# orjfickel/Small-Project-UV-Robot-Ray-Tracer

Hardware: AMD Instinct MI355X
Metric: Mray/s (extend+shade) on C046_1.glb 1920x1080x8-bounce (higher is better)
Workload: dtype f32; 1 GPU; testroomopt.glb (stand-in for the absent rooms/C046_1.glb), 2073600 photons/launch x 8 waves, lamp 0 of lange_route.xml, SEED_0=0; step = reset + generate + extend of all waves (batched), accumulate + shade replayed per wave + sync; triangles=44866, mode=batched, launch_pipelining=True, flavour=0, seed_mode=0, wide_bvh=False, parallelism=1 GPU, self_comm=False, high_priority_stream=False, full=False

## Files before the change

include/uvrt.h:

```cpp
#ifndef UVRT_H
#define UVRT_H

#include <stdint.h>

#ifdef __cplusplus
extern "C" {
#endif

typedef struct uvrt_ctx uvrt_ctx;

enum {
    UVRT_OK = 0,
    UVRT_ERR_INVALID = -1,
    UVRT_ERR_HIP = -2,
    UVRT_ERR_NO_DEVICE = -3,
    UVRT_ERR_BVH = -4,
    UVRT_ERR_STACK = -5
};

enum { UVRT_MAP_SUM = 0, UVRT_MAP_MAX = 1 };

const char* uvrt_last_error(void);
const char* uvrt_version(void);

// ... 96 lines not shown
int32_t uvrt_dedupe_classes_default(void);
int uvrt_batch_deposits(uvrt_ctx* ctx, int64_t* out);
int uvrt_batch_residue(uvrt_ctx* ctx, int64_t* nonzero);
int uvrt_dedupe_classes(const float lamp[3], int32_t count, const uint32_t* seed_prev, const uint32_t* seed_next,
                        int32_t seed_mode, int64_t first_gid, int64_t n, int32_t max_classes, uint32_t* class_masks,
                        int32_t* class_count, int64_t* deposits);
int uvrt_set_helper_priority(uvrt_ctx* ctx, int32_t prio);
int uvrt_get_helper_priority(uvrt_ctx* ctx, int32_t* prio);
int uvrt_batch_traced_rays(uvrt_ctx* ctx, int64_t* out);
uint32_t uvrt_seed_input(int64_t gid, const float lamp[3], uint32_t seed_prev, uint32_t seed_next, int32_t seed_mode);
int uvrt_dedupe_plan(const float lamp[3], int32_t count, const uint32_t* seed_prev, const uint32_t* seed_next,
                     int32_t seed_mode, int64_t first_gid, int64_t n, uint32_t* masks);
int uvrt_dedupe_plan_tiled(const float lamp[3], int32_t count, const uint32_t* seed_prev, const uint32_t* seed_next,
                           int32_t seed_mode, int64_t first_gid, int64_t n, int32_t tile_keys, int64_t chunk_first,
                           int64_t chunk_n, uint32_t* masks);
int uvrt_dedupe_mark_device(uvrt_ctx* ctx, const float lamp[3], int32_t count, const uint32_t* seed_prev,
                            const uint32_t* seed_next, int32_t seed_mode, int64_t first_gid, int64_t n, int64_t chunk_first,
                            int64_t chunk_n, uint32_t* masks, uint32_t* block_owner_counts);

int uvrt_comm_available(void);
int uvrt_comm_unique_id(void* id128);
int uvrt_comm_init_rank(uvrt_ctx* ctx, const void* id128, int32_t rank, int32_t world);
int uvrt_comm_init_all(uvrt_ctx** ctxs, int32_t n);
int uvrt_comm_destroy(uvrt_ctx* ctx);
int uvrt_comm_info(uvrt_ctx* ctx, int32_t out4[4]);
int uvrt_reduce_batch(uvrt_ctx* ctx);
int uvrt_reduce_batch_group(uvrt_ctx** ctxs, int32_t n);

enum { UVRT_PLAN_CONVERGED = 0, UVRT_PLAN_ITERATION_CAP = 1 };
typedef struct {
// ... 84 lines not shown
```

small-project-uv-robot-ray-tracer_amd/capi.py:

```python
from __future__ import annotations

import ctypes as C
import os

import numpy as np

_HERE = os.path.dirname(os.path.abspath(__file__))
LIB_PATH = os.path.join(_HERE, "libuvrt_hip.so")
LIB_DEV_PATH = os.path.join(_HERE, "libuvrt_hip_dev.so")

RAY_DT = np.dtype([("dirx", "<f4"), ("diry", "<f4"), ("dirz", "<f4"),
                   ("origx", "<f4"), ("origy", "<f4"), ("origz", "<f4"),
                   ("dist", "<f4"), ("triID", "<u4")])

MAP_SUM, MAP_MAX = 0, 1

_vp, _i32, _i64, _f32, _u32 = C.c_void_p, C.c_int32, C.c_int64, C.c_float, C.c_uint32
_fp = C.POINTER(C.c_float)
SYMBOLS = [
    ("uvrt_last_error", C.c_char_p, []),
    ("uvrt_version", C.c_char_p, []),
    ("uvrt_create", C.c_int, [C.c_int, C.POINTER(_vp)]),
    ("uvrt_destroy", None, [_vp]),
    ("uvrt_set_stream", C.c_int, [_vp, _vp]),
# ... 18 lines not shown
    ("uvrt_fold_batch", C.c_int, [_vp]),
    ("uvrt_read_batch_counts", C.c_int, [_vp, _i32, _vp, _i32, _i32]),
    ("uvrt_set_dedupe", C.c_int, [_vp, _i32]),
    ("uvrt_set_helper_priority", C.c_int, [_vp, _i32]),
    ("uvrt_get_helper_priority", C.c_int, [_vp, C.POINTER(_i32)]),
    ("uvrt_batch_traced_rays", C.c_int, [_vp, C.POINTER(_i64)]),
    ("uvrt_set_dedupe_classes", C.c_int, [_vp, _i32]),
    ("uvrt_get_dedupe_classes", C.c_int, [_vp, C.POINTER(_i32)]),
    ("uvrt_dedupe_classes_default", _i32, []),
    ("uvrt_batch_deposits", C.c_int, [_vp, C.POINTER(_i64)]),
    ("uvrt_batch_residue", C.c_int, [_vp, C.POINTER(_i64)]),
    ("uvrt_dedupe_classes", C.c_int, [_fp, _i32, _vp, _vp, _i32, _i64, _i64, _i32, _vp, C.POINTER(_i32), C.POINTER(_i64)]),
    ("uvrt_seed_input", _u32, [_i64, _fp, _u32, _u32, _i32]),
    ("uvrt_dedupe_plan", C.c_int, [_fp, _i32, _vp, _vp, _i32, _i64, _i64, _vp]),
    ("uvrt_dedupe_plan_tiled", C.c_int, [_fp, _i32, _vp, _vp, _i32, _i64, _i64, _i32, _i64, _i64, _vp]),
    ("uvrt_dedupe_mark_device", C.c_int, [_vp, _fp, _i32, _vp, _vp, _i32, _i64, _i64, _i64, _i64, _vp, _vp]),
    ("uvrt_comm_available", C.c_int, []),
    ("uvrt_comm_info", C.c_int, [_vp, C.POINTER(_i32)]),
    ("uvrt_comm_unique_id", C.c_int, [_vp]),
    ("uvrt_comm_init_rank", C.c_int, [_vp, _vp, _i32, _i32]),
    ("uvrt_comm_init_all", C.c_int, [C.POINTER(_vp), _i32]),
    ("uvrt_comm_destroy", C.c_int, [_vp]),
    ("uvrt_reduce_batch", C.c_int, [_vp]),
    ("uvrt_reduce_batch_group", C.c_int, [C.POINTER(_vp), _i32]),
    ("uvrt_advance_seed", C.c_int, [_vp, _fp, _f32]),
    ("uvrt_set_seed_mode", C.c_int, [_vp, _i32]),
    ("uvrt_seed_next_mode", _u32, [_fp, _f32, _u32, _i32]),
    ("uvrt_set_sort_bits", C.c_int, [_vp, _i32]),
    ("uvrt_set_record_hits", C.c_int, [_vp, _i32]),
    ("uvrt_set_flavour", C.c_int, [_vp, _i32]),
# ... 172 lines not shown
    sn = np.ascontiguousarray(seed_next_, dtype=np.uint32)
    assert sp.size == sn.size
    max_classes = dedupe_classes_default() if max_classes is None else max_classes
    out = np.zeros(DEDUPE_CLASS_MAX, dtype=np.uint32)
    nc, dep = _i32(), _i64()
    rc = lib().uvrt_dedupe_classes(_f3(lamp), int(sp.size), _ptr(sp), _ptr(sn), int(seed_mode), int(first_gid), int(n),
                                   int(max_classes), _ptr(out), C.byref(nc), C.byref(dep))
    if rc != 0:
        raise UvrtError("uvrt error %d: %s" % (rc, lib().uvrt_last_error().decode()))
    return out[:int(nc.value)].copy(), int(dep.value)


DEDUPE_CLASS_MAX = 32
DEDUPE_CLASS_LAUNCHES = 30
DEDUPE_TILE_KEYS = 3840
DEDUPE_BLOCK_GIDS = 2048


def dedupe_plan_tiled(lamp, seed_prev, seed_next_, seed_mode, first_gid, n, tile_keys=DEDUPE_TILE_KEYS, chunk_first=None,
                      chunk_n=None):
    sp = np.ascontiguousarray(seed_prev, dtype=np.uint32)
    sn = np.ascontiguousarray(seed_next_, dtype=np.uint32)
    assert sp.size == sn.size
    chunk_first = first_gid if chunk_first is None else chunk_first
    chunk_n = n if chunk_n is None else chunk_n
    out = np.empty((sp.size, int(chunk_n)), dtype=np.uint32)
    rc = lib().uvrt_dedupe_plan_tiled(_f3(lamp), int(sp.size), _ptr(sp), _ptr(sn), int(seed_mode), int(first_gid), int(n),
                                      int(tile_keys), int(chunk_first), int(chunk_n), _ptr(out))
    if rc != 0:
        raise UvrtError("uvrt error %d: %s" % (rc, lib().uvrt_last_error().decode()))
    return out


def seed_next_sweep(frm, light_length, seed_prev):
    return int(lib().uvrt_seed_next_sweep(_f3(frm), float(np.float32(light_length)), int(seed_prev)))


def comm_unique_id():
    buf = C.create_string_buffer(128)
    rc = lib().uvrt_comm_unique_id(buf)
    if rc != 0:
        raise UvrtError("uvrt error %d: %s" % (rc, lib().uvrt_last_error().decode()))
    return buf.raw
# ... 463 lines not shown
```

small-project-uv-robot-ray-tracer_amd/csrc/uvrt_capi.hip:

```cpp
#include "uvrt_ctx.h"

using namespace uvrt;
using namespace uvrt_impl;

namespace uvrt_impl {

thread_local std::string g_err;

int fail(int code, const char* fmt, ...)
{
    char buf[512];
    va_list ap;
    va_start(ap, fmt);
    vsnprintf(buf, sizeof buf, fmt, ap);
    va_end(ap);
    g_err = buf;
    return code;
}

}

uvrt_ctx::~uvrt_ctx()
{
    plan_drop(this);
// ... 74 lines not shown
        if (l > 0) HIP_TRY(hipStreamCreateWithFlags(&c->lanes[l].side, hipStreamNonBlocking));
        HIP_TRY(hipEventCreateWithFlags(&c->lanes[l].ev_tail, hipEventDisableTiming));
    }
    HIP_TRY(hipEventCreateWithFlags(&c->ev_fence, hipEventDisableTiming));
    HIP_TRY(hipEventCreateWithFlags(&c->ev_mapfence, hipEventDisableTiming));
    if (const char* e = getenv("UVRT_LANES")) { const int v = atoi(e); if (v >= 1 && v <= uvrt_ctx::MAXL) c->nlanes = v; }
    if (const char* e = getenv("UVRT_PIPELINE")) c->pipeline = atoi(e) != 0;
    if (const char* e = getenv("UVRT_BATCH_CHUNK_MB")) { const long v = atol(e); if (v > 0) c->batch_chunk_bytes = c->dedupe_chunk_bytes = (size_t)v << 20; }
#ifdef UVRT_DEV_VARIANTS
    if (const char* e = getenv("UVRT_PROBE_SKIP_GENERATE")) c->probe_skip_generate = atoi(e);
    if (const char* e = getenv("UVRT_NEARFAR_MINMAX")) c->nearfar_minmax = atoi(e) != 0;
#endif
    if (const char* e = getenv("UVRT_DRAIN_MERGE")) c->drain_merge = atoi(e) != 0;
    if (const char* e = getenv("UVRT_DEDUPE")) c->dedupe = atoi(e) != 0;
    if (const char* e = getenv("UVRT_DEDUPE_CLASSES")) { const int v = atoi(e); if (v >= 0 && v <= DEDUPE_CLASS_MAX) c->dedupe_classes = v; }
    if (const char* e = getenv("UVRT_DEDUPE_CLASS_REPLICAS")) { const int v = atoi(e); if (v >= 1 && v <= 16) c->dedupe_class_replicas = v; }
    if (const char* e = getenv("UVRT_DEDUPE_CLASS_MB")) { const long v = atol(e); if (v > 0 && v <= 4096) c->dedupe_class_bytes = (size_t)v << 20; }
    if (const char* e = getenv("UVRT_HELPER_PRIO")) { const int v = atoi(e); if (v >= 0 && v <= 3) c->helper_prio = v; }
    if (const char* e = getenv("UVRT_BATCH_LANES")) { const int v = atoi(e); if (v >= 1 && v <= uvrt_ctx::MAXL - 1) c->batch_lanes = v; }
    if (const char* e = getenv("UVRT_COMM_RESERVE_CUS")) { const int v = atoi(e); if (v >= 0 && v <= 64 && v % 8 == 0) c->comm_reserve_knob = v; }
    if (const char* e = getenv("UVRT_HOT_SAMPLE")) { const int v = atoi(e); if (v >= 256 && v <= (1 << 20)) c->hot_sample = v; }
    if (const char* e = getenv("UVRT_HOT_DIRECT")) { const int v = atoi(e); if (v >= 0 && v <= 8192) c->hot_direct = v; }
    if (const char* e = getenv("UVRT_HOT_TAIL")) { const int v = atoi(e); if (v >= 0 && v < 64) c->hot_tail = v; }
    if (int rc = c->error_flag.ensure(256, true, c->stream)) return rc;
#ifndef UVRT_TRIP_STATS
    void* dp = nullptr;
    HIP_TRY(hipHostMalloc((void**)&c->host_flag, 64, hipHostMallocMapped | hipHostMallocCoherent));
    HIP_TRY(hipHostGetDevicePointer(&dp, c->host_flag, 0));
    memset(c->host_flag, 0, 64);
    c->host_flag_dev = (uint32_t*)dp;
// ... 624 lines not shown
```

small-project-uv-robot-ray-tracer_amd/csrc/uvrt_capi_batch.hip:

```cpp
#include "uvrt_ctx.h"

using namespace uvrt;
using namespace uvrt_impl;

namespace uvrt_impl {

static int trace_launches(uvrt_ctx* c, const uvrt_launch* launches, float light_length, int32_t count, int64_t first_gid,
                          int64_t n, const char* who)
{
    if (!c || !launches || !c->have_scene) return fail(UVRT_ERR_INVALID, "%s: null argument or no scene", who);
    if (count <= 0 || count > MAX_BATCH) return fail(UVRT_ERR_INVALID, "%s: count must be in [1,%d]", who, MAX_BATCH);
    if (n <= 0 || first_gid < 0 || first_gid + n > (int64_t)INT32_MAX)
        return fail(UVRT_ERR_INVALID, "%s: bad global-id range", who);
    if (c->b_count > 0) return fail(UVRT_ERR_INVALID, "%s: the previous batch has not been replayed (uvrt_replay_batch)", who);
    if (c->record_hits || c->sort_bits != 0)
        return fail(UVRT_ERR_INVALID, "%s: per-ray hit records and ray ordering are per-launch features", who);
    int nsweeps = 0;
    for (int k = 0; k < count; ++k) {
        if (launches[k].kind != UVRT_LAUNCH_STOP && launches[k].kind != UVRT_LAUNCH_SWEEP)
            return fail(UVRT_ERR_INVALID, "%s: launch %d: kind must be UVRT_LAUNCH_STOP or UVRT_LAUNCH_SWEEP", who, k);
        nsweeps += launches[k].kind == UVRT_LAUNCH_SWEEP;
    }
    if (nsweeps > 0 && c->seed_mode != 0)
        return fail(UVRT_ERR_INVALID, "%s: seed mode 1 models the SEED race of generate.cl only; a sweep needs "
// ... 247 lines not shown
            for (int64_t g0 = 0; g0 < n; g0 += pc.chunk_gids) {
                const int64_t gn = std::min(pc.chunk_gids, n - g0);
                const int ph0 = gfirst[g] + pc.k0;
                hipStream_t ls;
                if (int rcl = next_chunk_lane(&ls)) return rcl;
                const size_t at = (size_t)ph0 * (size_t)n_pad + (size_t)pc.kc * (size_t)g0;
                GenDedupeParams dq;
                memset(&dq, 0, sizeof dq);
                dq.g = pc.G;
                dq.rays = S.rays.as<float4>() + at;
                dq.masks = S.masks.as<uint32_t>() + at;
                dq.total = S.dd_counts.as<uint32_t>() + dd_used;
                dq.deposits = S.dd_counts.as<uint32_t>() + dd_chunks + dd_used++;
                dq.cls = pc.cls;
                dq.tmp = cur_lane(c).dd_tmp.as<uint32_t>();
                dq.block_counts = cur_lane(c).dd_blocks.as<uint32_t>();
                dq.g0 = first_gid + g0;
                dq.gn = gn;
                dedupe_tile_range(dq.g, dq.g0, dq.gn, DEDUPE_TILE_KEYS, dq.key_lo, dq.tiles);
                dq.light_length = light_length;
                dq.prio = c->helper_prio;
                launch_generate_dedupe(dq, ls);
                if (int rcl = lane_stream(c, &ls)) return rcl;
                ExtendParams p;
                fill_launch(c, p, gx[g], gz[g]);
                p.rays = dq.rays;
                p.masks = dq.masks;
                p.n_dev = dq.total;
                p.counts = S.planes.as<int32_t>() + (size_t)ph0 * plane_ints;
                p.count_replicas = R;
                p.count_stride = c->T;
                p.n = (int64_t)pc.kc * gn;
                p.plane_stride = (uint32_t)plane_ints;
                p.cls_replicas = pc.cls.count > 0 ? cls_repl : 0;
// ... 201 lines not shown
        return fail(UVRT_ERR_INVALID, "%s: null argument, or count outside [2,%d]", who, DEDUPE_MAX);
    memset(&G, 0, sizeof G);
    G.lx = lamp[0]; G.ly = lamp[1]; G.lz = lamp[2];
    G.seed_mode = seed_mode;
    G.count = count;
    G.first_gid = first_gid; G.n = n;
    for (int j = 0; j < count; ++j) { G.seed_prev[j] = seed_prev[j]; G.seed_next[j] = seed_next[j]; }
    if (!dedupe_group_ok(G)) return fail(UVRT_ERR_INVALID, "%s: these launches cannot form a dedupe group", who);
    return UVRT_OK;
}
static bool chunk_ok(const DedupeGroup& G, int64_t chunk_first, int64_t chunk_n)
{
    return chunk_n > 0 && chunk_first >= G.first_gid && chunk_first + chunk_n <= G.first_gid + G.n;
}

int uvrt_dedupe_plan_tiled(const float lamp[3], int32_t count, const uint32_t* seed_prev, const uint32_t* seed_next,
                           int32_t seed_mode, int64_t first_gid, int64_t n, int32_t tile_keys, int64_t chunk_first,
                           int64_t chunk_n, uint32_t* masks)
{
    DedupeGroup G;
    if (int rc = hook_group(G, "uvrt_dedupe_plan_tiled", lamp, count, seed_prev, seed_next, seed_mode, first_gid, n)) return rc;
    if (!masks || tile_keys <= 0 || !chunk_ok(G, chunk_first, chunk_n))
        return fail(UVRT_ERR_INVALID, "uvrt_dedupe_plan_tiled: null masks, no tile width, or a chunk outside the range");
    std::vector<uint32_t> table((size_t)tile_keys);
    dedupe_plan_tiled(G, tile_keys, chunk_first, chunk_n, table.data(), masks);
    return UVRT_OK;
}

int32_t uvrt_dedupe_classes_default(void) { return DEDUPE_CLASSES_DEFAULT; }

int uvrt_dedupe_classes(const float lamp[3], int32_t count, const uint32_t* seed_prev, const uint32_t* seed_next, int32_t seed_mode,
                        int64_t first_gid, int64_t n, int32_t max_classes, uint32_t* class_masks, int32_t* class_count,
                        int64_t* deposits)
{
    DedupeGroup G;
    if (int rc = hook_group(G, "uvrt_dedupe_classes", lamp, count, seed_prev, seed_next, seed_mode, first_gid, n)) return rc;
    if (!class_masks || !class_count || max_classes < 0 || max_classes > DEDUPE_CLASS_MAX)
        return fail(UVRT_ERR_INVALID, "uvrt_dedupe_classes: null output, or a maximum outside [0,%d]", DEDUPE_CLASS_MAX);
    std::vector<uint32_t> table((size_t)DEDUPE_TILE_KEYS);
    DedupeTally cand[DEDUPE_CLASS_MAX];
    int nc = 0;
// ... 15 lines not shown
{
    if (!c) return fail(UVRT_ERR_INVALID, "uvrt_dedupe_mark_device: null context");
    GenDedupeParams dq;
    memset(&dq, 0, sizeof dq);
    if (int rc = hook_group(dq.g, "uvrt_dedupe_mark_device", lamp, count, seed_prev, seed_next, seed_mode, first_gid, n)) return rc;
    if (!masks || !block_owner_counts || !chunk_ok(dq.g, chunk_first, chunk_n))
        return fail(UVRT_ERR_INVALID, "uvrt_dedupe_mark_device: null output, or a chunk outside the range");
    if (int rc = set_device(c)) return rc;
    if (int rc = join_all(c)) return rc;
    Lane& L = c->lanes[0];
    const size_t nblocks = (size_t)count * (size_t)((chunk_n + DD_SLOTS - 1) / DD_SLOTS);
    HIP_TRY(hipStreamSynchronize(c->stream));
    if (int rc = L.dd_tmp.ensure((size_t)count * (size_t)chunk_n * 4, false, c->stream)) return rc;
    if (int rc = L.dd_blocks.ensure((size_t)count * (size_t)((chunk_n + 255) / 256) * 4, true, c->stream)) return rc;
    dq.tmp = L.dd_tmp.as<uint32_t>();
    dq.block_counts = L.dd_blocks.as<uint32_t>();
    dq.g0 = chunk_first;
    dq.gn = chunk_n;
    dedupe_tile_range(dq.g, dq.g0, dq.gn, DEDUPE_TILE_KEYS, dq.key_lo, dq.tiles);
    dq.prio = c->helper_prio;
    launch_dedupe_mark(dq, c->stream);
    HIP_TRY(hipGetLastError());
    HIP_TRY(hipMemcpyAsync(masks, dq.tmp, (size_t)count * (size_t)chunk_n * 4, hipMemcpyDeviceToHost, c->stream));
    HIP_TRY(hipMemcpyAsync(block_owner_counts, dq.block_counts, nblocks * 4, hipMemcpyDeviceToHost, c->stream));
    HIP_TRY(hipMemsetAsync(dq.block_counts, 0, nblocks * 4, c->stream));
    HIP_TRY(hipStreamSynchronize(c->stream));
    return UVRT_OK;
}

int uvrt_fold_batch(uvrt_ctx* c)
{
    if (!c || c->b_count <= 0) return fail(UVRT_ERR_INVALID, "uvrt_fold_batch: no traced batch");
    if (c->b_is_folded) return UVRT_OK;
    if (int rc = set_device(c)) return rc;
// ... 85 lines not shown
```

small-project-uv-robot-ray-tracer_amd/csrc/uvrt_ctx.h:

```cpp
#pragma once
#include "../../include/uvrt.h"
#include "uvrt_device.h"

#include <cmath>
#include <cstdarg>
#include <cstdio>
#include <cstring>
#include <memory>
#include <string>
#include <vector>

namespace uvrt_impl {

extern thread_local std::string g_err;
int fail(int code, const char* fmt, ...);

#define HIP_TRY(expr)                                                                   \
    do {                                                                                \
        hipError_t e_ = (expr);                                                         \
        if (e_ != hipSuccess)                                                           \
            return ::uvrt_impl::fail(UVRT_ERR_HIP, "%s failed: %s (%s:%d)", #expr,      \
                                     hipGetErrorString(e_), __FILE__, __LINE__);        \
    } while (0)

// ... 115 lines not shown
    uint64_t b_chunks = 0;
    int batch_lanes = 2;
    int32_t b_repl = 16;
    std::vector<DevBuf> b_recs;
    struct RecsKey {
        RecsTag tag; const uint32_t* perm = nullptr; uint64_t gen = 0;
        bool holds(float ox, float oz, const uint32_t* pm, uint64_t g) const { return tag.matches(ox, oz) && perm == pm && gen == g; }
    };
    std::vector<RecsKey> b_recs_key;
    int32_t b_count = 0;
    int64_t b_n = 0, b_npad = 0;
    int32_t b_phys[uvrt::MAX_BATCH] = {};
    int helper_prio = 1;
    bool dedupe = true;
    int64_t b_traced_known = -1;
    int32_t b_traced_chunks = 0;
    int32_t dedupe_classes = uvrt::DEDUPE_CLASSES_DEFAULT;
    int32_t dedupe_class_replicas = 4;
    size_t dedupe_class_bytes = (size_t)96 << 20;
    int32_t b_ncls = 0, b_cls_repl = 1;
    uint64_t b_cls_launches[uvrt::MAX_CLASS_PLANES] = {};
    bool b_is_folded = false;
    void* comm = nullptr;
    int comm_reserve_knob = 8;
    int lanes_masked_cus = 0;
    int comm_rank = 0, comm_world = 1;

    uint32_t seed = 0;
    int32_t seed_mode = 0;

// ... 286 lines not shown
```

small-project-uv-robot-ray-tracer_amd/csrc/uvrt_dedupe.h:

```cpp
#pragma once
#include <stdint.h>

#if defined(__HIPCC__)
#define UVRT_HD __host__ __device__ __forceinline__
#else
#define UVRT_HD inline
#endif

namespace uvrt {

constexpr int DEDUPE_MAX = 31;
constexpr int64_t DEDUPE_GID_END = 126322567;

UVRT_HD float seed_sum_of(int threadID, uint32_t SEED, float lx, float ly, float lz)
{
    float acc = (float)(int)((uint32_t)threadID * 17u + 1u);
    acc = acc + lx * 13.0f;
    acc = acc + ly * 7.0f;
    acc = acc + lz * 11.0f;
    acc = acc + (float)(SEED >> 15);
    return acc;
}
UVRT_HD float seed_sum(int64_t gid, float lx, float ly, float lz, uint32_t seed_prev, uint32_t seed_next, int32_t seed_mode)
{
// ... 10 lines not shown
    float lx, ly, lz;
    int32_t seed_mode;
    int32_t count;
    int64_t first_gid, n;
    uint32_t seed_prev[DEDUPE_MAX], seed_next[DEDUPE_MAX];
    int32_t offset[DEDUPE_MAX];
    int32_t key0[DEDUPE_MAX];
};

UVRT_HD int32_t dedupe_key(const DedupeGroup& G, int j, int64_t gid)
{
    const int32_t s = (int32_t)seed_sum(gid, G.lx, G.ly, G.lz, G.seed_prev[j], G.seed_next[j], G.seed_mode);
    return (G.seed_mode == 1 && s < 0) ? 0 : s;
}

UVRT_HD int32_t dedupe_key1(const DedupeGroup& G, int j, int32_t gid)
{
    const int32_t s = (int32_t)seed_sum_of(gid, G.seed_mode == 1 ? G.seed_prev[j] : G.seed_next[j], G.lx, G.ly, G.lz);
    return (G.seed_mode == 1 && s < 0) ? 0 : s;
}

UVRT_HD int32_t dedupe_find(const DedupeGroup& G, int j, int32_t t, int32_t lo, int32_t last, int32_t& g)
{
    g = g < lo ? lo : (g > last ? last : g);
    int32_t v = dedupe_key1(G, j, g);
    while (v > t && g > lo) v = dedupe_key1(G, j, --g);
    while (v < t && g < last) v = dedupe_key1(G, j, ++g);
    return v;
}
UVRT_HD int32_t dedupe_estimate(const DedupeGroup& G, int j, int32_t t)
{
    return (int32_t)((float)((int64_t)t - (int64_t)G.offset[j]) * (1.0f / 17.0f));
}

UVRT_HD int dedupe_multiplicity(const DedupeGroup& G, int j, int32_t t, int32_t g)
// ... 55 lines not shown
        }
    }
    while (b - a > 1) {
        const int32_t m = a + (b - a) / 2;
        if ((int64_t)dedupe_key1(G, j, m) >= t) b = m; else a = m;
    }
    return b;
}

UVRT_HD void dedupe_tile_run(const DedupeGroup& G, int j, int64_t t0, int32_t W, int32_t& g_lo, int32_t& g_hi)
{
    const int32_t lo = (int32_t)(G.first_gid > 1 ? G.first_gid : 1), hi = (int32_t)(G.first_gid + G.n);
    g_lo = dedupe_lower_bound(G, j, t0, lo, hi);
    g_hi = dedupe_lower_bound(G, j, t0 + W, g_lo, hi);
}
UVRT_HD bool dedupe_tile_holds_gid0(const DedupeGroup& G, int j, int64_t t0, int32_t W)
{
    return G.first_gid == 0 && (int64_t)G.key0[j] >= t0 && (int64_t)G.key0[j] < t0 + W;
}
UVRT_HD uint32_t dedupe_tile_slot(int32_t key, int64_t t0) { return (uint32_t)key - (uint32_t)(int32_t)t0; }

UVRT_HD void dedupe_tile_insert(uint32_t* table, uint32_t slot, int j)
{
    const uint32_t bit = 1u << j;
#if defined(__HIP_DEVICE_COMPILE__)
    if (atomicOr(&table[slot], bit) & bit) atomicOr(&table[slot], DEDUPE_MANY);
#else
    if (table[slot] & bit) table[slot] |= DEDUPE_MANY;
    table[slot] |= bit;
#endif
}
UVRT_HD uint32_t dedupe_tile_resolve(uint32_t entry, int k)
{
    if (entry & DEDUPE_MANY) return 1u << k;
// ... 4 lines not shown
UVRT_HD void dedupe_tile_range(const DedupeGroup& G, int64_t c0, int64_t cn, int32_t W, int64_t& key_lo, int64_t& tiles)
{
    int64_t kmin = INT64_MAX, kmax = INT64_MIN;
    const int64_t last = c0 + cn - 1, lo1 = c0 > 1 ? c0 : 1;
    for (int j = 0; j < G.count; ++j) {
        int64_t e[3];
        int ne = 0;
        if (c0 == 0) e[ne++] = G.key0[j];
        if (lo1 <= last) { e[ne++] = dedupe_key1(G, j, (int32_t)lo1); e[ne++] = dedupe_key1(G, j, (int32_t)last); }
        for (int i = 0; i < ne; ++i) { kmin = e[i] < kmin ? e[i] : kmin; kmax = e[i] > kmax ? e[i] : kmax; }
    }
    key_lo = kmin;
    tiles = cn > 0 ? (kmax - kmin) / W + 1 : 0;
}

inline void dedupe_plan_tiled(const DedupeGroup& G, int32_t W, int64_t c0, int64_t cn, uint32_t* table, uint32_t* masks)
{
    int64_t key_lo, tiles;
    dedupe_tile_range(G, c0, cn, W, key_lo, tiles);
    for (int64_t tile = 0; tile < tiles; ++tile) {
        const int64_t t0 = key_lo + tile * W;
        int32_t g_lo[DEDUPE_MAX], g_hi[DEDUPE_MAX];
        for (int32_t i = 0; i < W; ++i) table[i] = 0u;
        for (int j = 0; j < G.count; ++j) {
            dedupe_tile_run(G, j, t0, W, g_lo[j], g_hi[j]);
            for (int32_t g = g_lo[j]; g < g_hi[j]; ++g) dedupe_tile_insert(table, dedupe_tile_slot(dedupe_key1(G, j, g), t0), j);
            if (dedupe_tile_holds_gid0(G, j, t0, W)) dedupe_tile_insert(table, dedupe_tile_slot(G.key0[j], t0), j);
        }
        for (int k = 0; k < G.count; ++k) {
            const int64_t a = g_lo[k] > c0 ? g_lo[k] : c0, b = g_hi[k] < c0 + cn ? g_hi[k] : c0 + cn;
            for (int64_t g = a; g < b; ++g)
                masks[(int64_t)k * cn + (g - c0)] = dedupe_tile_resolve(table[dedupe_tile_slot(dedupe_key1(G, k, (int32_t)g), t0)], k);
            if (c0 == 0 && dedupe_tile_holds_gid0(G, k, t0, W))
                masks[(int64_t)k * cn] = dedupe_tile_resolve(table[dedupe_tile_slot(G.key0[k], t0)], k);
        }
    }
}

constexpr int DEDUPE_CLASS_MAX = 32;
constexpr int DEDUPE_CLASSES_DEFAULT = 32;
constexpr int DEDUPE_CLASS_SLOTS = 64;
constexpr int DEDUPE_CLASS_LAUNCHES = 30;
constexpr uint32_t DEDUPE_PLANE_FORM = 1u << 30, DEDUPE_CLASS_FORM = 1u << 29, DEDUPE_PLANE_INDEX = 0xFFFFu;
// ... 164 lines not shown
```

small-project-uv-robot-ray-tracer_amd/csrc/uvrt_device.h:

```cpp
#pragma once
#include <hip/hip_runtime.h>
#include <stdint.h>
#include "uvrt_dedupe.h"

namespace uvrt {

constexpr uint32_t REF_LEAF_BIT = 0x80000000u;
constexpr uint32_t REF_DONE = 0xFFFFFFFFu;
constexpr uint32_t REF_FIRST_MASK = 0x07FFFFFFu;
constexpr int REF_COUNT_SHIFT = 27;
constexpr int MAX_TRIS = 1 << 27;

struct alignas(16) PairRec {
    float4 c0min_ref0;
    float4 c0max_ref1;
    float4 c1min;
    float4 c1max;
};

struct alignas(16) LeafTri {
    float4 v0_id;
    float4 e1;
    float4 e2;
};
// ... 109 lines not shown
    float lx[MAX_BATCH], ly[MAX_BATCH], lz[MAX_BATCH];
    uint32_t seed_prev[MAX_BATCH], seed_next[MAX_BATCH];
    int32_t prio;
};

constexpr int DD_ROUNDS = 8, DD_SLOTS = 256 * DD_ROUNDS;
struct GenDedupeParams {
    DedupeGroup g;
    float4* rays;
    uint32_t* masks;
    uint32_t* total;
    uint32_t* tmp;
    uint32_t* block_counts;
    int64_t g0, gn;
    int64_t key_lo, tiles;
    float light_length;
    int32_t prio;
    uint32_t* deposits;
    DedupeClasses cls;
};
void launch_generate_dedupe(const GenDedupeParams& p, hipStream_t s);
void launch_dedupe_mark(const GenDedupeParams& p, hipStream_t s);
struct ExtendParams;
bool launch_extend6_dedupe(const ExtendParams& p, int code, int grid_per_cu, hipStream_t s);

struct ReplayOp {
    int32_t plane;
    float duration;
    int32_t shade;
    int32_t which_map;
// ... 212 lines not shown
```

small-project-uv-robot-ray-tracer_amd/csrc/uvrt_kernels.hip:

```cpp
#include "uvrt_device.h"

namespace uvrt {


__device__ __forceinline__ uint32_t coherence_key(uint32_t qphi, uint32_t qy, uint32_t qo,
                                                  int bphi, int by, int bo)
{
    uint32_t key = 0;
    while (bphi > 0 || by > 0 || bo > 0) {
        if (bphi > 0) { --bphi; key = (key << 1) | ((qphi >> bphi) & 1u); }
        if (by > 0) { --by; key = (key << 1) | ((qy >> by) & 1u); }
        if (bo > 0) { --bo; key = (key << 1) | ((qo >> bo) & 1u); }
    }
    return key;
}

__global__ __launch_bounds__(256) void k_generate(GenParams p)
{
    helper_priority(p.prio);
    if (blockIdx.x >= p.ray_blocks) {
        const int j = (int)(blockIdx.x - p.ray_blocks) * 256 + threadIdx.x;
        if (j < p.prep_npairs) prepare_record6(p.prep_pairs, p.prep_recs, p.lx, p.lz, p.prep_npairs, j, p.prep_perm);
        return;
    }
// ... 21 lines not shown
    }
}

__global__ __launch_bounds__(256) void k_generate_batch(GenBatchParams p)
{
    helper_priority(p.prio);
    const int64_t i = (int64_t)blockIdx.x * 256 + threadIdx.x;
    if (i >= p.n) return;
    const int k = blockIdx.y;
    float r0;
    double x, y;
    p.rays[(int64_t)k * p.n_pad + i] = generate_ray(p.lx[k], p.ly[k], p.lz[k], p.light_length, p.first_gid + i,
                                                    p.seed_prev[k], p.seed_next[k], p.seed_mode, r0, x, y);
}

__global__ __launch_bounds__(256) void k_dedupe_mark(GenDedupeParams p)
{
    helper_priority(p.prio);
    constexpr int32_t W = DEDUPE_TILE_KEYS;
    __shared__ uint32_t s_table[W];
    __shared__ int32_t s_run[DEDUPE_MAX][2];
    __shared__ uint32_t s_cnt[DEDUPE_MAX * 2];
    const int tid = threadIdx.x, K = p.g.count;
    const int64_t t0 = p.key_lo + (int64_t)blockIdx.x * W;
    const uint32_t nb = (uint32_t)((p.gn + DD_SLOTS - 1) / DD_SLOTS);
    for (int i = tid; i < W; i += 256) s_table[i] = 0u;
    if (tid < 2 * K) s_cnt[tid] = 0u;
    if (tid < K) {
        int32_t g_lo, g_hi;
        dedupe_tile_run(p.g, tid, t0, W, g_lo, g_hi);
        s_run[tid][0] = g_lo;
        s_run[tid][1] = g_hi;
    }
    __syncthreads();
    for (int j = 0; j < K; ++j) {
        const int32_t hi = s_run[j][1];
        for (int32_t g = s_run[j][0] + tid; g < hi; g += 256) {
            const uint32_t slot = dedupe_tile_slot(dedupe_key1(p.g, j, g), t0);
            if (slot < (uint32_t)W) dedupe_tile_insert(s_table, slot, j);
        }
    }
    if (tid < K && dedupe_tile_holds_gid0(p.g, tid, t0, W)) dedupe_tile_insert(s_table, dedupe_tile_slot(p.g.key0[tid], t0), tid);
    __syncthreads();
    const int32_t c0 = (int32_t)p.g0, c1 = (int32_t)(p.g0 + p.gn);
    for (int j = 0; j < K; ++j) {
        const int32_t a = max(s_run[j][0], c0), b = min(s_run[j][1], c1);
        const uint32_t b0 = (uint32_t)(a - c0) / (uint32_t)DD_SLOTS;
        for (int32_t base = a; base < b; base += 256) {
            const int32_t g = base + tid;
            uint32_t mask = 0u, rel = 0u;
            if (g < b) {
                const uint32_t slot = dedupe_tile_slot(dedupe_key1(p.g, j, g), t0);
                mask = dedupe_tile_resolve(slot < (uint32_t)W ? s_table[slot] : DEDUPE_MANY, j);
                p.tmp[(int64_t)j * p.gn + (g - c0)] = mask;
                rel = (uint32_t)(g - c0) / (uint32_t)DD_SLOTS - b0;
            }
            const uint32_t n0 = (uint32_t)__popcll(__builtin_amdgcn_ballot_w64(mask != 0u && rel == 0u));
            const uint32_t n1 = (uint32_t)__popcll(__builtin_amdgcn_ballot_w64(mask != 0u && rel == 1u));
            if ((tid & 63) == 0) {
                if (n0) atomicAdd(&s_cnt[2 * j], n0);
                if (n1) atomicAdd(&s_cnt[2 * j + 1], n1);
            }
            if (mask != 0u && rel >= 2u) atomicAdd(&p.block_counts[(size_t)j * nb + b0 + rel], 1u);
        }
    }
    if (c0 == 0 && tid < K && dedupe_tile_holds_gid0(p.g, tid, t0, W)) {
        const uint32_t mask = dedupe_tile_resolve(s_table[dedupe_tile_slot(p.g.key0[tid], t0)], tid);
        p.tmp[(int64_t)tid * p.gn] = mask;
        if (mask != 0u) atomicAdd(&p.block_counts[(size_t)tid * nb], 1u);
    }
    __syncthreads();
    if (tid < 2 * K && s_cnt[tid] != 0u) {
        const int j = tid >> 1;
        const uint32_t b0 = (uint32_t)(max(s_run[j][0], c0) - c0) / (uint32_t)DD_SLOTS;
        atomicAdd(&p.block_counts[(size_t)j * nb + b0 + (uint32_t)(tid & 1)], s_cnt[tid]);
    }
}

__global__ __launch_bounds__(256) void k_dedupe_scan(uint32_t* block_counts, uint32_t* total, uint32_t* deposits, uint32_t nblocks, int prio)
{
    helper_priority(prio);
    __shared__ uint32_t s_part[256];
    const uint32_t tid = threadIdx.x;
    if (tid == 0u) *deposits = 0u;
    const uint32_t per = (nblocks + 255u) / 256u;
    const uint32_t lo = min(tid * per, nblocks), hi = min(lo + per, nblocks);
    uint32_t sum = 0;
    for (uint32_t b = lo; b < hi; ++b) sum += block_counts[b];
    s_part[tid] = sum;
    __syncthreads();
    for (uint32_t off = 1; off < 256u; off <<= 1) {
// ... 446 lines not shown
    GenParams p = p0;
    p.ray_blocks = p.n > 0 ? blocks_for(p.n, 256) : 0u;
    const unsigned prep_blocks = p.prep_recs ? blocks_for(p.prep_npairs, 256) : 0u;
    if (p.ray_blocks + prep_blocks == 0) return;
    hipLaunchKernelGGL(k_generate, dim3(p.ray_blocks + prep_blocks), dim3(256), 0, s, p);
}

void launch_generate_batch(const GenBatchParams& p, hipStream_t s)
{
    if (p.n <= 0 || p.count <= 0) return;
    hipLaunchKernelGGL(k_generate_batch, dim3(blocks_for(p.n, 256), (unsigned)p.count), dim3(256), 0, s, p);
}

void launch_dedupe_mark(const GenDedupeParams& p, hipStream_t s)
{
    if (p.gn <= 0 || p.g.count <= 0 || p.tiles <= 0) return;
    hipLaunchKernelGGL(k_dedupe_mark, dim3((unsigned)p.tiles), dim3(256), 0, s, p);
}

void launch_generate_dedupe(const GenDedupeParams& p, hipStream_t s)
{
    if (p.gn <= 0 || p.g.count <= 0) return;
    const dim3 grid(blocks_for(p.gn, DD_SLOTS), (unsigned)p.g.count);
    launch_dedupe_mark(p, s);
    hipLaunchKernelGGL(k_dedupe_scan, dim3(1), dim3(256), 0, s, p.block_counts, p.total, p.deposits, grid.x * grid.y, (int)p.prio);
    hipLaunchKernelGGL(k_dedupe_write, grid, dim3(256), 0, s, p);
}

void launch_fold_planes(int32_t* planes, int32_t* folded, int32_t nplanes, int32_t replicas, int32_t T, int prio, hipStream_t s)
{
    if (nplanes <= 0 || T <= 0) return;
    hipLaunchKernelGGL(k_fold_planes, dim3(blocks_for((int64_t)T * 4, 256), (unsigned)nplanes), dim3(256), 0, s, planes,
// ... 112 lines not shown
```

Baseline: 16100 Mray/s.

## Restructure dedupe mark kernel into single-wave strips of smaller key tiles

The dedupe mark kernel now runs one 64-lane wave per block over a strip of several consecutive 960-key tiles, in place of one 256-thread block per 3840-key tile. Each strip does a single binary search and then advances each ray run incrementally from tile to tile. Duplicate detection compares neighbouring keys inside the run rather than going through table collisions, and per-block owner counts are gathered in registers and flushed with fewer atomics. The aim is to remove repeated binary searches and shared-memory and atomic overhead, at the cost of less parallelism per block and more serial work within each strip.

```diff
diff --git a/include/uvrt.h b/include/uvrt.h
--- a/include/uvrt.h
+++ b/include/uvrt.h
@@ -134,6 +134,9 @@
 int uvrt_dedupe_plan_tiled(const float lamp[3], int32_t count, const uint32_t* seed_prev, const uint32_t* seed_next,
                            int32_t seed_mode, int64_t first_gid, int64_t n, int32_t tile_keys, int64_t chunk_first,
                            int64_t chunk_n, uint32_t* masks);
+int uvrt_dedupe_plan_strips(const float lamp[3], int32_t count, const uint32_t* seed_prev, const uint32_t* seed_next,
+                            int32_t seed_mode, int64_t first_gid, int64_t n, int32_t tile_keys, int32_t strip_tiles,
+                            int64_t chunk_first, int64_t chunk_n, uint32_t* masks);
 int uvrt_dedupe_mark_device(uvrt_ctx* ctx, const float lamp[3], int32_t count, const uint32_t* seed_prev,
                             const uint32_t* seed_next, int32_t seed_mode, int64_t first_gid, int64_t n, int64_t chunk_first,
                             int64_t chunk_n, uint32_t* masks, uint32_t* block_owner_counts);
diff --git a/small-project-uv-robot-ray-tracer_amd/capi.py b/small-project-uv-robot-ray-tracer_amd/capi.py
--- a/small-project-uv-robot-ray-tracer_amd/capi.py
+++ b/small-project-uv-robot-ray-tracer_amd/capi.py
@@ -56,6 +56,7 @@
     ("uvrt_seed_input", _u32, [_i64, _fp, _u32, _u32, _i32]),
     ("uvrt_dedupe_plan", C.c_int, [_fp, _i32, _vp, _vp, _i32, _i64, _i64, _vp]),
     ("uvrt_dedupe_plan_tiled", C.c_int, [_fp, _i32, _vp, _vp, _i32, _i64, _i64, _i32, _i64, _i64, _vp]),
+    ("uvrt_dedupe_plan_strips", C.c_int, [_fp, _i32, _vp, _vp, _i32, _i64, _i64, _i32, _i32, _i64, _i64, _vp]),
     ("uvrt_dedupe_mark_device", C.c_int, [_vp, _fp, _i32, _vp, _vp, _i32, _i64, _i64, _i64, _i64, _vp, _vp]),
     ("uvrt_comm_available", C.c_int, []),
     ("uvrt_comm_info", C.c_int, [_vp, C.POINTER(_i32)]),
@@ -258,19 +259,25 @@
 DEDUPE_CLASS_MAX = 32
 DEDUPE_CLASS_LAUNCHES = 30
 DEDUPE_TILE_KEYS = 3840
+DEDUPE_MARK_KEYS = 960
+DEDUPE_STRIP_TILES = 4
 DEDUPE_BLOCK_GIDS = 2048
 
 
 def dedupe_plan_tiled(lamp, seed_prev, seed_next_, seed_mode, first_gid, n, tile_keys=DEDUPE_TILE_KEYS, chunk_first=None,
-                      chunk_n=None):
+                      chunk_n=None, strip_tiles=None):
     sp = np.ascontiguousarray(seed_prev, dtype=np.uint32)
     sn = np.ascontiguousarray(seed_next_, dtype=np.uint32)
     assert sp.size == sn.size
     chunk_first = first_gid if chunk_first is None else chunk_first
     chunk_n = n if chunk_n is None else chunk_n
     out = np.empty((sp.size, int(chunk_n)), dtype=np.uint32)
-    rc = lib().uvrt_dedupe_plan_tiled(_f3(lamp), int(sp.size), _ptr(sp), _ptr(sn), int(seed_mode), int(first_gid), int(n),
-                                      int(tile_keys), int(chunk_first), int(chunk_n), _ptr(out))
+    if strip_tiles is None:
+        rc = lib().uvrt_dedupe_plan_tiled(_f3(lamp), int(sp.size), _ptr(sp), _ptr(sn), int(seed_mode), int(first_gid), int(n),
+                                          int(tile_keys), int(chunk_first), int(chunk_n), _ptr(out))
+    else:
+        rc = lib().uvrt_dedupe_plan_strips(_f3(lamp), int(sp.size), _ptr(sp), _ptr(sn), int(seed_mode), int(first_gid), int(n),
+                                           int(tile_keys), int(strip_tiles), int(chunk_first), int(chunk_n), _ptr(out))
     if rc != 0:
         raise UvrtError("uvrt error %d: %s" % (rc, lib().uvrt_last_error().decode()))
     return out
diff --git a/small-project-uv-robot-ray-tracer_amd/csrc/uvrt_capi.hip b/small-project-uv-robot-ray-tracer_amd/csrc/uvrt_capi.hip
--- a/small-project-uv-robot-ray-tracer_amd/csrc/uvrt_capi.hip
+++ b/small-project-uv-robot-ray-tracer_amd/csrc/uvrt_capi.hip
@@ -112,6 +112,7 @@
     if (const char* e = getenv("UVRT_DRAIN_MERGE")) c->drain_merge = atoi(e) != 0;
     if (const char* e = getenv("UVRT_DEDUPE")) c->dedupe = atoi(e) != 0;
     if (const char* e = getenv("UVRT_DEDUPE_CLASSES")) { const int v = atoi(e); if (v >= 0 && v <= DEDUPE_CLASS_MAX) c->dedupe_classes = v; }
+    if (const char* e = getenv("UVRT_DEDUPE_STRIP")) { const int v = atoi(e); if (v >= 1 && v <= 1024) c->dedupe_strip = v; }
     if (const char* e = getenv("UVRT_DEDUPE_CLASS_REPLICAS")) { const int v = atoi(e); if (v >= 1 && v <= 16) c->dedupe_class_replicas = v; }
     if (const char* e = getenv("UVRT_DEDUPE_CLASS_MB")) { const long v = atol(e); if (v > 0 && v <= 4096) c->dedupe_class_bytes = (size_t)v << 20; }
     if (const char* e = getenv("UVRT_HELPER_PRIO")) { const int v = atoi(e); if (v >= 0 && v <= 3) c->helper_prio = v; }
diff --git a/small-project-uv-robot-ray-tracer_amd/csrc/uvrt_capi_batch.hip b/small-project-uv-robot-ray-tracer_amd/csrc/uvrt_capi_batch.hip
--- a/small-project-uv-robot-ray-tracer_amd/csrc/uvrt_capi_batch.hip
+++ b/small-project-uv-robot-ray-tracer_amd/csrc/uvrt_capi_batch.hip
@@ -4,6 +4,13 @@
 using namespace uvrt_impl;
 
 namespace uvrt_impl {
+
+static void mark_tiles(const uvrt_ctx* c, GenDedupeParams& q)
+{
+    dedupe_tile_range(q.g, q.g0, q.gn, DEDUPE_MARK_KEYS, q.key_lo, q.tiles);
+    const int64_t fit = std::min<int64_t>(2 * DEDUPE_STRIP_TILES, std::max<int64_t>(DEDUPE_STRIP_TILES, q.tiles / 4096));
+    q.strip_tiles = c->dedupe_strip > 0 ? c->dedupe_strip : (int32_t)fit;
+}
 
 static int trace_launches(uvrt_ctx* c, const uvrt_launch* launches, float light_length, int32_t count, int64_t first_gid,
                           int64_t n, const char* who)
@@ -285,10 +292,10 @@
                 dq.deposits = S.dd_counts.as<uint32_t>() + dd_chunks + dd_used++;
                 dq.cls = pc.cls;
                 dq.tmp = cur_lane(c).dd_tmp.as<uint32_t>();
-                dq.block_counts = cur_lane(c).dd_blocks.as<uint32_t>();
                 dq.g0 = first_gid + g0;
                 dq.gn = gn;
-                dedupe_tile_range(dq.g, dq.g0, dq.gn, DEDUPE_TILE_KEYS, dq.key_lo, dq.tiles);
+                dq.block_counts = cur_lane(c).dd_blocks.as<uint32_t>();
+                mark_tiles(c, dq);
                 dq.light_length = light_length;
                 dq.prio = c->helper_prio;
                 launch_generate_dedupe(dq, ls);
@@ -520,17 +527,25 @@
     return chunk_n > 0 && chunk_first >= G.first_gid && chunk_first + chunk_n <= G.first_gid + G.n;
 }
 
+int uvrt_dedupe_plan_strips(const float lamp[3], int32_t count, const uint32_t* seed_prev, const uint32_t* seed_next,
+                            int32_t seed_mode, int64_t first_gid, int64_t n, int32_t tile_keys, int32_t strip_tiles,
+                            int64_t chunk_first, int64_t chunk_n, uint32_t* masks)
+{
+    DedupeGroup G;
+    if (int rc = hook_group(G, "uvrt_dedupe_plan_tiled", lamp, count, seed_prev, seed_next, seed_mode, first_gid, n)) return rc;
+    if (!masks || tile_keys <= 0 || strip_tiles <= 0 || !chunk_ok(G, chunk_first, chunk_n))
+        return fail(UVRT_ERR_INVALID, "uvrt_dedupe_plan_tiled: null masks, no tile width, no strip length, or a chunk outside the range");
+    std::vector<uint32_t> table((size_t)tile_keys);
+    dedupe_plan_tiled(G, tile_keys, strip_tiles, chunk_first, chunk_n, table.data(), masks);
+    return UVRT_OK;
+}
+
 int uvrt_dedupe_plan_tiled(const float lamp[3], int32_t count, const uint32_t* seed_prev, const uint32_t* seed_next,
                            int32_t seed_mode, int64_t first_gid, int64_t n, int32_t tile_keys, int64_t chunk_first,
                            int64_t chunk_n, uint32_t* masks)
 {
-    DedupeGroup G;
-    if (int rc = hook_group(G, "uvrt_dedupe_plan_tiled", lamp, count, seed_prev, seed_next, seed_mode, first_gid, n)) return rc;
-    if (!masks || tile_keys <= 0 || !chunk_ok(G, chunk_first, chunk_n))
-        return fail(UVRT_ERR_INVALID, "uvrt_dedupe_plan_tiled: null masks, no tile width, or a chunk outside the range");
-    std::vector<uint32_t> table((size_t)tile_keys);
-    dedupe_plan_tiled(G, tile_keys, chunk_first, chunk_n, table.data(), masks);
-    return UVRT_OK;
+    return uvrt_dedupe_plan_strips(lamp, count, seed_prev, seed_next, seed_mode, first_gid, n, tile_keys, DEDUPE_STRIP_TILES, chunk_first,
+                                   chunk_n, masks);
 }
 
 int32_t uvrt_dedupe_classes_default(void) { return DEDUPE_CLASSES_DEFAULT; }
@@ -576,10 +591,10 @@
     if (int rc = L.dd_tmp.ensure((size_t)count * (size_t)chunk_n * 4, false, c->stream)) return rc;
     if (int rc = L.dd_blocks.ensure((size_t)count * (size_t)((chunk_n + 255) / 256) * 4, true, c->stream)) return rc;
     dq.tmp = L.dd_tmp.as<uint32_t>();
-    dq.block_counts = L.dd_blocks.as<uint32_t>();
     dq.g0 = chunk_first;
     dq.gn = chunk_n;
-    dedupe_tile_range(dq.g, dq.g0, dq.gn, DEDUPE_TILE_KEYS, dq.key_lo, dq.tiles);
+    dq.block_counts = L.dd_blocks.as<uint32_t>();
+    mark_tiles(c, dq);
     dq.prio = c->helper_prio;
     launch_dedupe_mark(dq, c->stream);
     HIP_TRY(hipGetLastError());
diff --git a/small-project-uv-robot-ray-tracer_amd/csrc/uvrt_ctx.h b/small-project-uv-robot-ray-tracer_amd/csrc/uvrt_ctx.h
--- a/small-project-uv-robot-ray-tracer_amd/csrc/uvrt_ctx.h
+++ b/small-project-uv-robot-ray-tracer_amd/csrc/uvrt_ctx.h
@@ -153,6 +153,7 @@
     int helper_prio = 1;
     bool dedupe = true;
     int64_t b_traced_known = -1;
+    int32_t dedupe_strip = 0;
     int32_t b_traced_chunks = 0;
     int32_t dedupe_classes = uvrt::DEDUPE_CLASSES_DEFAULT;
     int32_t dedupe_class_replicas = 4;
diff --git a/small-project-uv-robot-ray-tracer_amd/csrc/uvrt_dedupe.h b/small-project-uv-robot-ray-tracer_amd/csrc/uvrt_dedupe.h
--- a/small-project-uv-robot-ray-tracer_amd/csrc/uvrt_dedupe.h
+++ b/small-project-uv-robot-ray-tracer_amd/csrc/uvrt_dedupe.h
@@ -48,11 +48,13 @@
     return (G.seed_mode == 1 && s < 0) ? 0 : s;
 }
 
-UVRT_HD int32_t dedupe_key1(const DedupeGroup& G, int j, int32_t gid)
-{
-    const int32_t s = (int32_t)seed_sum_of(gid, G.seed_mode == 1 ? G.seed_prev[j] : G.seed_next[j], G.lx, G.ly, G.lz);
+UVRT_HD uint32_t dedupe_seed1(const DedupeGroup& G, int j) { return G.seed_mode == 1 ? G.seed_prev[j] : G.seed_next[j]; }
+UVRT_HD int32_t dedupe_key1_of(const DedupeGroup& G, uint32_t seed1, int32_t gid)
+{
+    const int32_t s = (int32_t)seed_sum_of(gid, seed1, G.lx, G.ly, G.lz);
     return (G.seed_mode == 1 && s < 0) ? 0 : s;
 }
+UVRT_HD int32_t dedupe_key1(const DedupeGroup& G, int j, int32_t gid) { return dedupe_key1_of(G, dedupe_seed1(G, j), gid); }
 
 UVRT_HD int32_t dedupe_find(const DedupeGroup& G, int j, int32_t t, int32_t lo, int32_t last, int32_t& g)
 {
@@ -138,10 +140,11 @@
     g_lo = dedupe_lower_bound(G, j, t0, lo, hi);
     g_hi = dedupe_lower_bound(G, j, t0 + W, g_lo, hi);
 }
-UVRT_HD bool dedupe_tile_holds_gid0(const DedupeGroup& G, int j, int64_t t0, int32_t W)
-{
-    return G.first_gid == 0 && (int64_t)G.key0[j] >= t0 && (int64_t)G.key0[j] < t0 + W;
-}
+UVRT_HD bool dedupe_tile_holds_key0(const DedupeGroup& G, int32_t key0, int64_t t0, int32_t W)
+{
+    return G.first_gid == 0 && (int64_t)key0 >= t0 && (int64_t)key0 < t0 + W;
+}
+UVRT_HD bool dedupe_tile_holds_gid0(const DedupeGroup& G, int j, int64_t t0, int32_t W) { return dedupe_tile_holds_key0(G, G.key0[j], t0, W); }
 UVRT_HD uint32_t dedupe_tile_slot(int32_t key, int64_t t0) { return (uint32_t)key - (uint32_t)(int32_t)t0; }
 
 UVRT_HD void dedupe_tile_insert(uint32_t* table, uint32_t slot, int j)
@@ -176,19 +179,51 @@
     tiles = cn > 0 ? (kmax - kmin) / W + 1 : 0;
 }
 
-inline void dedupe_plan_tiled(const DedupeGroup& G, int32_t W, int64_t c0, int64_t cn, uint32_t* table, uint32_t* masks)
+constexpr int32_t DEDUPE_MARK_KEYS = 960;
+constexpr int32_t DEDUPE_STRIP_TILES = 4;
+
+UVRT_HD bool dedupe_in_tile(int32_t key, int64_t t0, int32_t W) { return dedupe_tile_slot(key, t0) < (uint32_t)W; }
+UVRT_HD bool dedupe_run_twice(const DedupeGroup& G, uint32_t seed1, int32_t g, int32_t key, int32_t lo, int32_t hi)
+{
+    const int before = (g > lo) & (dedupe_key1_of(G, seed1, g - 1) == key), after = (g + 1 < hi) & (dedupe_key1_of(G, seed1, g + 1) == key);
+    return (before | after) != 0;
+}
+UVRT_HD void dedupe_tile_insert_run(uint32_t* table, uint32_t slot, int j, bool twice)
+{
+    const uint32_t v = (1u << j) | (twice ? DEDUPE_MANY : 0u);
+#if defined(__HIP_DEVICE_COMPILE__)
+    atomicOr(&table[slot], v);
+#else
+    table[slot] |= v;
+#endif
+}
+UVRT_HD int32_t dedupe_strip_first(const DedupeGroup& G, int j, int64_t t0)
+{
+    return dedupe_lower_bound(G, j, t0, (int32_t)(G.first_gid > 1 ? G.first_gid : 1), (int32_t)(G.first_gid + G.n));
+}
+
+inline void dedupe_plan_tiled(const DedupeGroup& G, int32_t W, int32_t strip, int64_t c0, int64_t cn, uint32_t* table, uint32_t* masks)
 {
     int64_t key_lo, tiles;
     dedupe_tile_range(G, c0, cn, W, key_lo, tiles);
+    const int32_t lo = (int32_t)(G.first_gid > 1 ? G.first_gid : 1), hi = (int32_t)(G.first_gid + G.n);
+    int32_t g_lo[DEDUPE_MAX], g_hi[DEDUPE_MAX];
     for (int64_t tile = 0; tile < tiles; ++tile) {
         const int64_t t0 = key_lo + tile * W;
-        int32_t g_lo[DEDUPE_MAX], g_hi[DEDUPE_MAX];
         for (int32_t i = 0; i < W; ++i) table[i] = 0u;
         for (int j = 0; j < G.count; ++j) {
-            dedupe_tile_run(G, j, t0, W, g_lo[j], g_hi[j]);
-            for (int32_t g = g_lo[j]; g < g_hi[j]; ++g) dedupe_tile_insert(table, dedupe_tile_slot(dedupe_key1(G, j, g), t0), j);
+            g_lo[j] = tile % strip == 0 ? dedupe_strip_first(G, j, t0) : g_hi[j];
+            const uint32_t seed1 = dedupe_seed1(G, j);
+            int32_t g = g_lo[j];
+            for (; g < hi; ++g) {
+                const int32_t key = dedupe_key1_of(G, seed1, g);
+                if (!dedupe_in_tile(key, t0, W)) break;
+                dedupe_tile_insert_run(table, dedupe_tile_slot(key, t0), j, dedupe_run_twice(G, seed1, g, key, lo, hi));
+            }
+            g_hi[j] = g;
+        }
+        for (int j = 0; j < G.count; ++j)
             if (dedupe_tile_holds_gid0(G, j, t0, W)) dedupe_tile_insert(table, dedupe_tile_slot(G.key0[j], t0), j);
-        }
         for (int k = 0; k < G.count; ++k) {
             const int64_t a = g_lo[k] > c0 ? g_lo[k] : c0, b = g_hi[k] < c0 + cn ? g_hi[k] : c0 + cn;
             for (int64_t g = a; g < b; ++g)
diff --git a/small-project-uv-robot-ray-tracer_amd/csrc/uvrt_device.h b/small-project-uv-robot-ray-tracer_amd/csrc/uvrt_device.h
--- a/small-project-uv-robot-ray-tracer_amd/csrc/uvrt_device.h
+++ b/small-project-uv-robot-ray-tracer_amd/csrc/uvrt_device.h
@@ -147,6 +147,7 @@
     uint32_t* block_counts;
     int64_t g0, gn;
     int64_t key_lo, tiles;
+    int32_t strip_tiles;
     float light_length;
     int32_t prio;
     uint32_t* deposits;
diff --git a/small-project-uv-robot-ray-tracer_amd/csrc/uvrt_kernels.hip b/small-project-uv-robot-ray-tracer_amd/csrc/uvrt_kernels.hip
--- a/small-project-uv-robot-ray-tracer_amd/csrc/uvrt_kernels.hip
+++ b/small-project-uv-robot-ray-tracer_amd/csrc/uvrt_kernels.hip
@@ -59,67 +59,95 @@
                                                     p.seed_prev[k], p.seed_next[k], p.seed_mode, r0, x, y);
 }
 
-__global__ __launch_bounds__(256) void k_dedupe_mark(GenDedupeParams p)
+__global__ __launch_bounds__(64) void k_dedupe_mark(GenDedupeParams p)
 {
     helper_priority(p.prio);
-    constexpr int32_t W = DEDUPE_TILE_KEYS;
+    constexpr int32_t W = DEDUPE_MARK_KEYS;
     __shared__ uint32_t s_table[W];
-    __shared__ int32_t s_run[DEDUPE_MAX][2];
-    __shared__ uint32_t s_cnt[DEDUPE_MAX * 2];
-    const int tid = threadIdx.x, K = p.g.count;
-    const int64_t t0 = p.key_lo + (int64_t)blockIdx.x * W;
+    const int lane = threadIdx.x, K = p.g.count;
     const uint32_t nb = (uint32_t)((p.gn + DD_SLOTS - 1) / DD_SLOTS);
-    for (int i = tid; i < W; i += 256) s_table[i] = 0u;
-    if (tid < 2 * K) s_cnt[tid] = 0u;
-    if (tid < K) {
-        int32_t g_lo, g_hi;
-        dedupe_tile_run(p.g, tid, t0, W, g_lo, g_hi);
-        s_run[tid][0] = g_lo;
-        s_run[tid][1] = g_hi;
-    }
-    __syncthreads();
-    for (int j = 0; j < K; ++j) {
-        const int32_t hi = s_run[j][1];
-        for (int32_t g = s_run[j][0] + tid; g < hi; g += 256) {
-            const uint32_t slot = dedupe_tile_slot(dedupe_key1(p.g, j, g), t0);
-            if (slot < (uint32_t)W) dedupe_tile_insert(s_table, slot, j);
-        }
-    }
-    if (tid < K && dedupe_tile_holds_gid0(p.g, tid, t0, W)) dedupe_tile_insert(s_table, dedupe_tile_slot(p.g.key0[tid], t0), tid);
-    __syncthreads();
+    const int32_t lo = (int32_t)(p.g.first_gid > 1 ? p.g.first_gid : 1), hi = (int32_t)(p.g.first_gid + p.g.n);
     const int32_t c0 = (int32_t)p.g0, c1 = (int32_t)(p.g0 + p.gn);
-    for (int j = 0; j < K; ++j) {
-        const int32_t a = max(s_run[j][0], c0), b = min(s_run[j][1], c1);
-        const uint32_t b0 = (uint32_t)(a - c0) / (uint32_t)DD_SLOTS;
-        for (int32_t base = a; base < b; base += 256) {
-            const int32_t g = base + tid;
-            uint32_t mask = 0u, rel = 0u;
-            if (g < b) {
-                const uint32_t slot = dedupe_tile_slot(dedupe_key1(p.g, j, g), t0);
-                mask = dedupe_tile_resolve(slot < (uint32_t)W ? s_table[slot] : DEDUPE_MANY, j);
-                p.tmp[(int64_t)j * p.gn + (g - c0)] = mask;
-                rel = (uint32_t)(g - c0) / (uint32_t)DD_SLOTS - b0;
+    const int64_t tile0 = (int64_t)blockIdx.x * p.strip_tiles;
+    const int64_t tile1 = tile0 + p.strip_tiles < p.tiles ? tile0 + p.strip_tiles : p.tiles;
+    int32_t run_lo = hi, run_hi = hi, key0 = 0;
+    uint32_t seed1 = 0u;
+    if (lane < K) {
+        run_lo = dedupe_strip_first(p.g, lane, p.key_lo + tile0 * W);
+        seed1 = dedupe_seed1(p.g, lane);
+        key0 = p.g.key0[lane];
+    }
+    uint32_t cnt_block = 0u, cnt = 0u;
+    const auto add_owners = [&](int j, uint32_t block, uint32_t owners) { atomicAdd(&p.block_counts[(size_t)j * nb + block], owners); };
+    const auto count_owners = [&](int j, uint32_t block, uint32_t owners) {
+        if (lane == j && owners != 0u) {
+            if (block != cnt_block) {
+                if (cnt != 0u) add_owners(j, cnt_block, cnt);
+                cnt_block = block;
+                cnt = 0u;
             }
-            const uint32_t n0 = (uint32_t)__popcll(__builtin_amdgcn_ballot_w64(mask != 0u && rel == 0u));
-            const uint32_t n1 = (uint32_t)__popcll(__builtin_amdgcn_ballot_w64(mask != 0u && rel == 1u));
-            if ((tid & 63) == 0) {
-                if (n0) atomicAdd(&s_cnt[2 * j], n0);
-                if (n1) atomicAdd(&s_cnt[2 * j + 1], n1);
+            cnt += owners;
+        }
+    };
+    for (int64_t tile = tile0; tile < tile1; ++tile) {
+        const int64_t t0 = p.key_lo + tile * W;
+        static_assert(W % 64 == 0, "the wave zeroes the table in whole rounds");
+#pragma unroll
+        for (int i = 0; i < W; i += 64) s_table[i + lane] = 0u;
+        __syncthreads();
+        for (int j = 0; j < K; ++j) {
+            int32_t base = __builtin_amdgcn_readlane(run_lo, j);
+            const uint32_t seed = (uint32_t)__builtin_amdgcn_readlane((int)seed1, j);
+            for (;;) {
+                const int32_t g = base + lane;
+                bool in = false;
+                if (g < hi) {
+                    const int32_t key = dedupe_key1_of(p.g, seed, g);
+                    in = dedupe_in_tile(key, t0, W);
+                    if (in) dedupe_tile_insert_run(s_table, dedupe_tile_slot(key, t0), j, dedupe_run_twice(p.g, seed, g, key, lo, hi));
+                }
+                const int32_t n_in = (int32_t)__popcll(__builtin_amdgcn_ballot_w64(in));
+                base += n_in;
+                if (n_in < 64) break;
             }
-            if (mask != 0u && rel >= 2u) atomicAdd(&p.block_counts[(size_t)j * nb + b0 + rel], 1u);
-        }
-    }
-    if (c0 == 0 && tid < K && dedupe_tile_holds_gid0(p.g, tid, t0, W)) {
-        const uint32_t mask = dedupe_tile_resolve(s_table[dedupe_tile_slot(p.g.key0[tid], t0)], tid);
-        p.tmp[(int64_t)tid * p.gn] = mask;
-        if (mask != 0u) atomicAdd(&p.block_counts[(size_t)tid * nb], 1u);
-    }
-    __syncthreads();
-    if (tid < 2 * K && s_cnt[tid] != 0u) {
-        const int j = tid >> 1;
-        const uint32_t b0 = (uint32_t)(max(s_run[j][0], c0) - c0) / (uint32_t)DD_SLOTS;
-        atomicAdd(&p.block_counts[(size_t)j * nb + b0 + (uint32_t)(tid & 1)], s_cnt[tid]);
-    }
+            if (lane == j) run_hi = base;
+        }
+        const bool holds0 = lane < K && dedupe_tile_holds_key0(p.g, key0, t0, W);
+        if (holds0) dedupe_tile_insert(s_table, dedupe_tile_slot(key0, t0), lane);
+        __syncthreads();
+        for (int j = 0; j < K; ++j) {
+            const int32_t a = max(__builtin_amdgcn_readlane(run_lo, j), c0), b = min(__builtin_amdgcn_readlane(run_hi, j), c1);
+            const uint32_t seed = (uint32_t)__builtin_amdgcn_readlane((int)seed1, j);
+            for (int32_t base = a; base < b; base += 64) {
+                const int32_t g = base + lane;
+                const uint32_t fb = (uint32_t)(base - c0) / (uint32_t)DD_SLOTS;
+                uint32_t mask = 0u, blk = fb;
+                if (g < b) {
+                    const uint32_t slot = dedupe_tile_slot(dedupe_key1_of(p.g, seed, g), t0);
+                    mask = dedupe_tile_resolve(slot < (uint32_t)W ? s_table[slot] : DEDUPE_MANY, j);
+                    p.tmp[(int64_t)j * p.gn + (g - c0)] = mask;
+                    blk = (uint32_t)(g - c0) / (uint32_t)DD_SLOTS;
+                }
+                const int32_t last = min(base + 63, b - 1);
+                if ((uint32_t)(last - c0) / (uint32_t)DD_SLOTS == fb) {
+                    count_owners(j, fb, (uint32_t)__popcll(__builtin_amdgcn_ballot_w64(mask != 0u)));
+                } else {
+                    const uint32_t n0 = (uint32_t)__popcll(__builtin_amdgcn_ballot_w64(mask != 0u && blk == fb));
+                    const uint32_t n1 = (uint32_t)__popcll(__builtin_amdgcn_ballot_w64(mask != 0u && blk != fb));
+                    count_owners(j, fb, n0);
+                    count_owners(j, fb + 1u, n1);
+                }
+            }
+        }
+        if (c0 == 0 && holds0) {
+            const uint32_t mask = dedupe_tile_resolve(s_table[dedupe_tile_slot(key0, t0)], lane);
+            p.tmp[(int64_t)lane * p.gn] = mask;
+            if (mask != 0u) add_owners(lane, 0u, 1u);
+        }
+        run_lo = run_hi;
+        __syncthreads();
+    }
+    if (lane < K && cnt != 0u) add_owners(lane, cnt_block, cnt);
 }
 
 __global__ __launch_bounds__(256) void k_dedupe_scan(uint32_t* block_counts, uint32_t* total, uint32_t* deposits, uint32_t nblocks, int prio)
@@ -596,8 +624,8 @@
 
 void launch_dedupe_mark(const GenDedupeParams& p, hipStream_t s)
 {
-    if (p.gn <= 0 || p.g.count <= 0 || p.tiles <= 0) return;
-    hipLaunchKernelGGL(k_dedupe_mark, dim3((unsigned)p.tiles), dim3(256), 0, s, p);
+    if (p.gn <= 0 || p.g.count <= 0 || p.tiles <= 0 || p.strip_tiles <= 0) return;
+    hipLaunchKernelGGL(k_dedupe_mark, dim3((unsigned)((p.tiles + p.strip_tiles - 1) / p.strip_tiles)), dim3(64), 0, s, p);
 }
 
 void launch_generate_dedupe(const GenDedupeParams& p, hipStream_t s)
```

Result: faster. 16540 Mray/s (median of 6 runs) (+2.7%).
